# peach-xiao/EMRT

Hardware: AMD Instinct MI355X
Metric: training tiles/sec at 256x256 (higher is better)
Workload: dtype bf16; 1 GPU; EMRT ResNet50, Potsdam 256x256, 6 classes, batch 8 per GPU, fwd+bwd+SGD step (BASELINE configs[1]), bf16; global_batch=8, parallelism=dp1, hipgraph=True

## Files before the change

### emrt_amd/csrc/norm.hip

```cpp
#include "common.hpp"
#include "bn_operand.hpp"
#include <stdlib.h>

using namespace emrt;

template <class T, int MODE>
__global__ __launch_bounds__(256) void col_reduce_kernel(const T* __restrict__ x, int ldx, const T* __restrict__ dy, int lddy,
                                                         const T* __restrict__ y, int ldy, const float* __restrict__ mean,
                                                         const float* __restrict__ invstd, long long M, int C, int tx_n,
                                                         float* __restrict__ partial, long long rpb, long long bs,
                                                         double* __restrict__ dsums, float* __restrict__ facc,
                                                         const float* __restrict__ mgamma = nullptr, const float* __restrict__ mbeta = nullptr) {
  __shared__ float red[256 * 8];
  const int ty_n = 256 / tx_n;
  const int tx = threadIdx.x % tx_n, ty = threadIdx.x / tx_n;
  const int c = (blockIdx.y * tx_n + tx) * 4;
  float s0[4] = {0, 0, 0, 0}, s1[4] = {0, 0, 0, 0};
  if (c < C) {
    float mu[4] = {0, 0, 0, 0}, is[4] = {1, 1, 1, 1};
    float msc[MODE == 3 ? 4 : 1], msh[MODE == 3 ? 4 : 1];
    if (MODE == 1 || MODE == 3) {
#pragma unroll
      for (int e = 0; e < 4; ++e) { mu[e] = mean[c + e]; is[e] = invstd[c + e]; }
      if constexpr (MODE == 3) {
#pragma unroll
        for (int e = 0; e < 4; ++e) bn_scale_shift(mu[e], is[e], mgamma[c + e], mbeta[c + e], msc[e], msh[e]);
      }
    }
    for (long long r = (long long)blockIdx.x * ty_n + ty; r < M; r += (long long)gridDim.x * ty_n) {
      float v[4];
      if (MODE == 0) {
        Vec4<T>::load(x + r * ldx + c, v);
#pragma unroll
        for (int e = 0; e < 4; ++e) { s0[e] += v[e]; s1[e] = fmaf(v[e], v[e], s1[e]); }
      } else if (MODE == 1 || MODE == 3) {
        const long long rs = (long long)gridDim.x * ty_n;
        float vv[4][4], gg[4][4], oo[4][4];
#pragma unroll
        for (int u = 0; u < 4; ++u) {
          const long long ru = r + u * rs < M ? r + u * rs : r;
          Vec4<T>::load(x + ru * ldx + c, vv[u]);
          Vec4<T>::load(dy + ru * lddy + c, gg[u]);
          if (y) Vec4<T>::load(y + ru * ldy + c, oo[u]);
        }
#pragma unroll
        for (int u = 0; u < 4; ++u) {
          const bool ok = r + u * rs < M;
#pragma unroll
          for (int e = 0; e < 4; ++e) {
            float g = ok ? gg[u][e] : 0.f;
            if (y) g = oo[u][e] > 0.f ? g : 0.f;
            if constexpr (MODE == 3) g = fmaf(vv[u][e], msc[e], msh[e]) > 0.f ? g : 0.f;
            s0[e] += g;
            s1[e] = fmaf(g, (vv[u][e] - mu[e]) * is[e], s1[e]);
          }
        }
        r += 3 * rs;
      } else {
        const long long bb = (M | rpb) <= 0xffffffffll ? (long long)((unsigned)r / (unsigned)rpb) : r / rpb;
        Vec4<T>::load(x + bb * bs + (r - bb * rpb) * ldx + c, v);
#pragma unroll
        for (int e = 0; e < 4; ++e) s0[e] += v[e];
      }
    }
  }
#pragma unroll
  for (int e = 0; e < 4; ++e) { red[threadIdx.x * 8 + e] = s0[e]; red[threadIdx.x * 8 + 4 + e] = s1[e]; }
  __syncthreads();
  if (ty == 0 && c < C) {
    for (int t = 1; t < ty_n; ++t) {
#pragma unroll
      for (int e = 0; e < 4; ++e) { s0[e] += red[(t * tx_n + tx) * 8 + e]; s1[e] += red[(t * tx_n + tx) * 8 + 4 + e]; }
    }
    if (dsums) {
      double* rep = dsums + (long long)(blockIdx.x & 7) * 2 * C;
#pragma unroll
      for (int e = 0; e < 4; ++e) { atomicAdd(rep + c + e, (double)s0[e]); atomicAdd(rep + C + c + e, (double)s1[e]); }
    } else if (facc) {
#pragma unroll
      for (int e = 0; e < 4; ++e)
        if (c + e < C) atomicAdd(facc + c + e, s0[e]);
    } else {
      float* pp = partial + (long long)blockIdx.x * 2 * C;
#pragma unroll
      for (int e = 0; e < 4; ++e) { pp[c + e] = s0[e]; pp[C + c + e] = s1[e]; }
    }
  }
}

static inline void col_reduce_geometry(long long M, int C, int& tx_n, int& gx, int& gy) {
  int quads = (C + 3) / 4;
  tx_n = 64;
  while (tx_n > 1 && tx_n / 2 >= quads) tx_n /= 2;
  gy = (quads + tx_n - 1) / tx_n;
  int ty_n = 256 / tx_n;
  long long want = (M + (long long)ty_n * 8 - 1) / ((long long)ty_n * 8);
  long long cap = 512 / gy;
  if (cap < 1) cap = 1;
  gx = (int)(want < 1 ? 1 : (want > cap ? cap : want));
}

__global__ __launch_bounds__(256) void bn_sum_partials_kernel(const float* __restrict__ partial, int nblk, int C, float* __restrict__ sums ) {
  __shared__ double red[8][33];
  const int cx = threadIdx.x & 31, py = threadIdx.x >> 5;
  const int c = blockIdx.x * 32 + cx;
  double s = 0.0;
  if (c < 2 * C)
    for (int b = py; b < nblk; b += 8) s += (double)partial[(long long)b * 2 * C + c];
  red[py][cx] = s;
  __syncthreads();
  if (py == 0 && c < 2 * C) {
    double t = 0.0;
#pragma unroll
    for (int k = 0; k < 8; ++k) t += red[k][cx];
    sums[c] = (float)t;
  }
}

__global__ __launch_bounds__(256) void partials_acc_kernel(const float* __restrict__ partial, int nblk, int C, float* __restrict__ dgamma,
                                                          float* __restrict__ dbeta) {
  __shared__ double red[8][33];
  const int cx = threadIdx.x & 31, py = threadIdx.x >> 5;
  const int c = blockIdx.x * 32 + cx;
  double s = 0.0;
  if (c < 2 * C)
    for (int b = py; b < nblk; b += 8) s += (double)partial[(long long)b * 2 * C + c];
  red[py][cx] = s;
  __syncthreads();
  if (py == 0 && c < 2 * C) {
    double t = 0.0;
#pragma unroll
    for (int k = 0; k < 8; ++k) t += red[k][cx];
    if (c < C) { if (dbeta) dbeta[c] += (float)t; }
    else if (dgamma) dgamma[c - C] += (float)t;
  }
}

__global__ void bn_bwd_finalize_kernel(const float* __restrict__ sums, int C, float* __restrict__ dgamma, float* __restrict__ dbeta) {
  const int c = blockIdx.x * blockDim.x + threadIdx.x;
  if (c >= C) return;
  if (dbeta) dbeta[c] += sums[c];
  if (dgamma) dgamma[c] += sums[C + c];
}

template <class T, bool JOIN = false>
__global__ __launch_bounds__(512) void bn_apply_kernel(const T* __restrict__ x, int ldx, const T* __restrict__ res, int ldres,
                                                       T* __restrict__ y, int ldy, const double* __restrict__ sums, double inv_count,
                                                       float eps, float momentum, float* __restrict__ mean_out,
                                                       float* __restrict__ invstd_out, float* __restrict__ run_mean,
                                                       float* __restrict__ run_var, const float* __restrict__ gamma,
                                                       const float* __restrict__ beta, long long M, int C, int relu, int rows_per_pass,
                                                       BnOperand rbn) {
  const int quads = C / 4;
  const int c = (threadIdx.x % quads) * 4;
  const int lane_row = threadIdx.x / quads;
  const long long rstep = (long long)gridDim.x * rows_per_pass;
  long long r = (long long)blockIdx.x * rows_per_pass + lane_row;
  float v[4], w[4];
  if (r < M) {
    Vec4<T>::load(x + r * ldx + c, v);
    if (res) Vec4<T>::load(res + r * ldres + c, w);
  }
  extern __shared__ float bn_lds[];
  if constexpr (JOIN) bn_operand_preamble(rbn, C, bn_lds + 2 * C, blockIdx.x == 0);
  for (int ch = threadIdx.x; ch < C; ch += blockDim.x) {
    const BnChan k = bn_chan(sums, run_mean, run_var, C, ch, inv_count, eps);
    float scale, shift;
    bn_scale_shift(k.mean, k.invstd, gamma[ch], beta[ch], scale, shift);
    bn_lds[ch] = scale;
    bn_lds[C + ch] = shift;
    if (sums && blockIdx.x == 0) {
      mean_out[ch] = k.mean;
      invstd_out[ch] = k.invstd;
      if (run_mean) {
        const double mu = rep_sum(sums, C, ch) * inv_count;
        double var = rep_sum(sums, C, C + ch) * inv_count - mu * mu;
        if (var < 0.0) var = 0.0;
        run_mean[ch] = momentum * run_mean[ch] + (1.f - momentum) * (float)mu;
        run_var[ch] = momentum * run_var[ch] + (1.f - momentum) * (float)var;
      }
// ... 589 lines not shown
__global__ __launch_bounds__(256) void gn_rows_stats_kernel(const T* __restrict__ x, int ldx, long long x_bs, GnRows gr, double* __restrict__ ws,
                                                            int N, int G) {
  __shared__ float red[256][2];
  int n, l, r0, r1, HW, row0;
  gn_rows_locate(gr, n, l, r0, r1, HW, row0);
  const int g = threadIdx.x % G, rl = threadIdx.x / G, nrl = 256 / G;
  const T* xp = x + (long long)n * x_bs + (long long)row0 * ldx + g * 8;
  float s0 = 0.f, s1 = 0.f;
  for (int p = r0 + rl; p < r1; p += nrl) {
    float v[8];
    Vec8<T>::load(xp + (long long)p * ldx, v);
#pragma unroll
    for (int e = 0; e < 8; ++e) { s0 += v[e]; s1 = fmaf(v[e], v[e], s1); }
  }
  red[threadIdx.x][0] = s0; red[threadIdx.x][1] = s1;
  __syncthreads();
  if ((int)threadIdx.x < 2 * G) {
    const int gg = threadIdx.x >> 1, w = threadIdx.x & 1;
    double a = 0.0;
    for (int t = 0; t < nrl; ++t) a += (double)red[t * G + gg][w];
    atomicAdd(&ws[(((long long)l * N + n) * G + gg) * 2 + w], a);
  }
}

template <class T>
__global__ __launch_bounds__(256) void gn_rows_apply_kernel(const T* __restrict__ x, int ldx, long long x_bs, const T* __restrict__ res, int ldres,
                                                            long long res_bs, T* __restrict__ out, int ldout, long long out_bs, GnRows gr,
                                                            const double* __restrict__ ws, float* __restrict__ mean_out,
                                                            float* __restrict__ rstd_out, int N, int G, float eps, int gelu) {
  int n, l, r0, r1, HW, row0;
  gn_rows_locate(gr, n, l, r0, r1, HW, row0);
  const int g = threadIdx.x % G, rl = threadIdx.x / G, nrl = 256 / G;
  const long long sidx = ((long long)l * N + n) * G + g;
  const double cnt = (double)HW * 8.0;
  const double mu_d = ws[sidx * 2] / cnt;
  double var = ws[sidx * 2 + 1] / cnt - mu_d * mu_d;
  if (var < 0.0) var = 0.0;
  const float mu = (float)mu_d, rs = (float)(1.0 / sqrt(var + (double)eps));
  if (mean_out && r0 == 0 && rl == 0) { mean_out[sidx] = mu; rstd_out[sidx] = rs; }
  const float* gam = gn_pick<0>(gr.lv.gamma, l) + g * 8;
  const float* bet = gn_pick<0>(gr.lv.beta, l) + g * 8;
  float sc[8], sh[8];
#pragma unroll
  for (int e = 0; e < 8; ++e) { sc[e] = rs * gam[e]; sh[e] = bet[e] - mu * sc[e]; }
  const T* xp = x + (long long)n * x_bs + (long long)row0 * ldx + g * 8;
  for (int p = r0 + rl; p < r1; p += nrl) {
    float v[8], o[8];
    Vec8<T>::load(xp + (long long)p * ldx, v);
#pragma unroll
    for (int e = 0; e < 8; ++e) {
      const float u = fmaf(v[e], sc[e], sh[e]);
      o[e] = gelu ? gelu_f(u) : u;
    }
    if (res) {
      float w[8];
      Vec8<T>::load(res + (long long)n * res_bs + (long long)(row0 + p) * ldres + g * 8, w);
#pragma unroll
      for (int e = 0; e < 8; ++e) o[e] += w[e];
    }
    Vec8<T>::store(out + (long long)n * out_bs + (long long)(row0 + p) * ldout + g * 8, o);
  }
}

template <class T>
__global__ __launch_bounds__(256) void gn_rows_bwd_stats_kernel(const T* __restrict__ x, int ldx, long long x_bs, const T* __restrict__ dy, int lddy,
                                                                long long dy_bs, GnRows gr, const float* __restrict__ mean,
                                                                const float* __restrict__ rstd, double* __restrict__ ws, int N, int G, int gelu) {
  __shared__ float chs[256][17];
  int n, l, r0, r1, HW, row0;
  gn_rows_locate(gr, n, l, r0, r1, HW, row0);
  const int g = threadIdx.x % G, rl = threadIdx.x / G, nrl = 256 / G;
  const long long sidx = ((long long)l * N + n) * G + g;
  const float mu = mean[sidx], rs = rstd[sidx];
  const float* gam = gn_pick<0>(gr.lv.gamma, l);
  const float* bet = gn_pick<0>(gr.lv.beta, l);
  float ga[8], be[8];
#pragma unroll
  for (int e = 0; e < 8; ++e) { ga[e] = gam[g * 8 + e]; be[e] = bet[g * 8 + e]; }
  const T* xp = x + (long long)n * x_bs + (long long)row0 * ldx + g * 8;
  const T* gp = dy + (long long)n * dy_bs + (long long)row0 * lddy + g * 8;
  float s0[8], s1[8];
#pragma unroll
  for (int e = 0; e < 8; ++e) { s0[e] = 0.f; s1[e] = 0.f; }
  for (int p = r0 + rl; p < r1; p += nrl) {
    float v[8], d[8];
    Vec8<T>::load(xp + (long long)p * ldx, v);
    Vec8<T>::load(gp + (long long)p * lddy, d);
#pragma unroll
    for (int e = 0; e < 8; ++e) {
      const float xh = (v[e] - mu) * rs;
      const float dd = gelu ? d[e] * gelu_grad_f(xh * ga[e] + be[e]) : d[e];
      s0[e] += dd;
      s1[e] = fmaf(dd, xh, s1[e]);
    }
  }
#pragma unroll
  for (int e = 0; e < 8; ++e) { chs[threadIdx.x][e] = s0[e]; chs[threadIdx.x][8 + e] = s1[e]; }
  __syncthreads();
  const int C = G * 8;
  if ((int)threadIdx.x < C) {
    const int c = threadIdx.x, gg = c >> 3, e = c & 7;
    float a = 0.f, b = 0.f;
    for (int t = 0; t < nrl; ++t) { a += chs[t * G + gg][e]; b += chs[t * G + gg][8 + e]; }
    float* dgam = nullptr; float* dbet = nullptr;
#pragma unroll
    for (int k = 0; k < GN_MAX_LEVELS; ++k)
      if (l == k) { dgam = gr.lv.dgamma[k]; dbet = gr.lv.dbeta[k]; }
    if (dbet) atomicAdd(dbet + c, a);
    if (dgam) atomicAdd(dgam + c, b);
    float wa = gam[c] * a, wb = gam[c] * b;
#pragma unroll
    for (int o = 1; o < 8; o <<= 1) { wa += __shfl_xor(wa, o, 64); wb += __shfl_xor(wb, o, 64); }
    if (e == 0) {
      const long long si = ((long long)l * N + n) * G + gg;
      atomicAdd(&ws[si * 2], (double)wa);
      atomicAdd(&ws[si * 2 + 1], (double)wb);
    }
  }
}

template <class T>
__global__ __launch_bounds__(256) void gn_rows_bwd_dx_kernel(const T* __restrict__ x, int ldx, long long x_bs, const T* __restrict__ dy, int lddy,
                                                             long long dy_bs, T* __restrict__ dx, int lddx, long long dx_bs, GnRows gr,
                                                             const float* __restrict__ mean, const float* __restrict__ rstd,
                                                             const double* __restrict__ ws, int N, int G, int gelu) {
  int n, l, r0, r1, HW, row0;
  gn_rows_locate(gr, n, l, r0, r1, HW, row0);
  const int g = threadIdx.x % G, rl = threadIdx.x / G, nrl = 256 / G;
  const long long sidx = ((long long)l * N + n) * G + g;
  const float mu = mean[sidx], rs = rstd[sidx];
  const double inv = 1.0 / ((double)HW * 8.0);
  const float A = (float)(ws[sidx * 2] * inv), Bq = (float)(ws[sidx * 2 + 1] * inv);
  const float* gam = gn_pick<0>(gr.lv.gamma, l) + g * 8;
  const float* bet = gn_pick<0>(gr.lv.beta, l) + g * 8;
  float ga[8], be[8];
#pragma unroll
  for (int e = 0; e < 8; ++e) { ga[e] = gam[e]; be[e] = bet[e]; }
  const T* xp = x + (long long)n * x_bs + (long long)row0 * ldx + g * 8;
  const T* gp = dy + (long long)n * dy_bs + (long long)row0 * lddy + g * 8;
  for (int p = r0 + rl; p < r1; p += nrl) {
    float v[8], d[8], o[8];
    Vec8<T>::load(xp + (long long)p * ldx, v);
    Vec8<T>::load(gp + (long long)p * lddy, d);
#pragma unroll
    for (int e = 0; e < 8; ++e) {
      const float xh = (v[e] - mu) * rs;
      const float dd = gelu ? d[e] * gelu_grad_f(xh * ga[e] + be[e]) : d[e];
      o[e] = rs * (ga[e] * dd - A - xh * Bq);
    }
    Vec8<T>::store(dx + (long long)n * dx_bs + (long long)(row0 + p) * lddx + g * 8, o);
  }
}

template <class T>
__global__ __launch_bounds__(256) void ln_fwd_kernel(const T* __restrict__ a, const T* __restrict__ b, const T* __restrict__ post,
                                                     T* __restrict__ z, T* __restrict__ out, const float* __restrict__ gamma,
                                                     const float* __restrict__ beta, float* __restrict__ mean_out,
                                                     float* __restrict__ rstd_out, long long rows, int C, float eps, float pdrop,
                                                     const unsigned long long* __restrict__ seed, unsigned salt,
                                                     const T* __restrict__ qpos, int qpos_rows, T* __restrict__ q_out) {
  const int lane = threadIdx.x & 63;
  const long long row = (long long)blockIdx.x * 4 + (threadIdx.x >> 6);
  if (row >= rows) return;
  const unsigned long long sd = pdrop > 0.f ? seed[0] : 0ull;
  const float ks = pdrop > 0.f ? 1.f / (1.f - pdrop) : 1.f;
  const int nq = C / 256 + ((C % 256) ? 1 : 0);
  float v[4][4];
  float s = 0.f;
  for (int j = 0; j < nq; ++j) {
    const int c = j * 256 + lane * 4;
    if (c < C) {
      Vec4<T>::load(a + row * C + c, v[j]);
      if (b) {
        float w[4];
        Vec4<T>::load(b + row * C + c, w);
        if (pdrop > 0.f) {
          uint32_t hq[2];
          drop_quad(sd, salt, (unsigned long long)(row * C + c) >> 2, hq);
          const uint32_t thr = drop_thr16(pdrop);
#pragma unroll
          for (int e = 0; e < 4; ++e) {
            const float d = drop_quad_keep(hq, e, thr) ? w[e] * ks : 0.f;
            w[e] = to_f32(from_f32<T>(d));
          }
        }
#pragma unroll
        for (int e = 0; e < 4; ++e) v[j][e] += w[e];
      }
      if (z) {
        Vec4<T>::store(z + row * C + c, v[j]);
        if (sizeof(T) == 2) {
#pragma unroll
          for (int e = 0; e < 4; ++e) v[j][e] = to_f32(from_f32<T>(v[j][e]));
        }
      }
#pragma unroll
      for (int e = 0; e < 4; ++e) s += v[j][e];
    }
  }
  const float mu = wave_sum(s) / (float)C;
// ... 113 lines not shown
#pragma unroll
        for (int k = 0; k < R; ++k) {
          if (!ok[k]) continue;
          float o[4];
#pragma unroll
          for (int e = 0; e < 4; ++e) o[e] = rs[k] * (gd[k][j][e] - s0[k] - xh[k][j][e] * s1[k]);
          if (addend) {
            float ad[4], oa[4];
            Vec4<T>::load(addend + row[k] * C + c, ad);
#pragma unroll
            for (int e = 0; e < 4; ++e) oa[e] = o[e] + ad[e];
            Vec4<T>::store(dz + row[k] * C + c, oa);
          } else {
            Vec4<T>::store(dz + row[k] * C + c, o);
          }
          if (dzb) {
            if (pdrop > 0.f) {
              uint32_t hq[2];
              drop_quad(sd, salt, (unsigned long long)(row[k] * C + c) >> 2, hq);
              const uint32_t thr = drop_thr16(pdrop);
#pragma unroll
              for (int e = 0; e < 4; ++e)
                o[e] = drop_quad_keep(hq, e, thr) ? to_f32(from_f32<T>(o[e])) * ks : 0.f;
            }
            Vec4<T>::store(dzb + row[k] * C + c, o);
          }
        }
      }
    }
  }
#pragma unroll
  for (int j = 0; j < NQ; ++j) {
    const int c = j * 256 + lane * 4;
    if (j < nq && c < C) {
#pragma unroll
      for (int e = 0; e < 4; ++e) { sm[(wv * 2 + 0) * C + c + e] = db[j][e]; sm[(wv * 2 + 1) * C + c + e] = dg[j][e]; }
    }
  }
  __syncthreads();
  for (int c = threadIdx.x; c < C; c += TPB) {
    float b0 = 0.f, g0 = 0.f;
    for (int w = 0; w < NWV; ++w) { b0 += sm[(w * 2 + 0) * C + c]; g0 += sm[(w * 2 + 1) * C + c]; }
    if (dgamma_direct || dbeta_direct) {
      if (dbeta_direct) atomicAdd(dbeta_direct + c, b0);
      if (dgamma_direct) atomicAdd(dgamma_direct + c, g0);
    } else {
      partial[(long long)blockIdx.x * 2 * C + c] = b0;
      partial[(long long)blockIdx.x * 2 * C + C + c] = g0;
    }
  }
}

extern "C" size_t emrt_colreduce_workspace_bytes(long long M, int C) {
  int tx, gx, gy;
  col_reduce_geometry(M, C, tx, gx, gy);
  return ((size_t)gx * 2 * C + 2 * (size_t)C) * sizeof(float);
}

static inline bool bn_rowgeom(long long M, int C, int& threads, int& rows_per_pass, int& grid) {
  const int quads = C / 4;
  if (quads <= 256) { if (256 % quads) return false; threads = 256; rows_per_pass = 256 / quads; }
  else if (quads <= 512) { threads = quads; rows_per_pass = 1; }
  else return false;
  const long long per_block = (long long)(g_tune.bn_block_kb > 0 ? g_tune.bn_block_kb : 8) * 1024;
  long long g = (M * C * 2 + per_block - 1) / per_block;
  const long long gmax = (M + rows_per_pass - 1) / rows_per_pass;
  if (g < 64) g = 64;
  if (g > 4096) g = 4096;
  if (g > gmax) g = gmax;
  if (g < 1) g = 1;
  grid = (int)g;
  return true;
}

extern "C" int emrt_bn_stats(const void* x, int ldx, long long M, int C, double* sums, int dtype, void* stream) {
  EMRT_REQUIRE_TRAIN_DTYPE(dtype);
  EMRT_REQUIRE(x && sums, "null pointer");
  EMRT_REQUIRE(C % 4 == 0 && ldx % 4 == 0, "C and ld must be multiples of 4");
  int tx, gx, gy;
  col_reduce_geometry(M, C, tx, gx, gy);
  hipStream_t st = (hipStream_t)stream;
  return with_train_dtype("emrt_bn_stats", dtype, [&](auto t) {
    using T = decltype(t);
    hipLaunchKernelGGL((col_reduce_kernel<T, 0>), dim3(gx, gy), dim3(256), 0, st, (const T*)x, ldx, nullptr, 0, nullptr, 0, nullptr, nullptr, M, C, tx, nullptr, M, 0LL, sums, nullptr);
    return check_launch("emrt_bn_stats");
  });
}

extern "C" int emrt_bn_apply(const void* x, int ldx, const void* res, int ldres, void* y, int ldy, const double* sums, double count,
                             float eps, float momentum, float* mean, float* invstd, float* run_mean, float* run_var,
                             const float* gamma, const float* beta, long long M, int C, int relu, int dtype, void* stream) {
  EMRT_REQUIRE_FWD_DTYPE(dtype);
  EMRT_REQUIRE(x && y && gamma && beta, "null pointer");
  EMRT_REQUIRE(sums ? (mean && invstd) : (run_mean && run_var), "training needs mean/invstd outputs, eval needs running statistics");
  EMRT_REQUIRE(C % 4 == 0 && ldx % 4 == 0 && ldy % 4 == 0 && (!res || ldres % 4 == 0), "C and ld must be multiples of 4");
  int threads, rpp, grid;
  EMRT_REQUIRE(bn_rowgeom(M, C, threads, rpp, grid), "unsupported channel count (C/4 must divide 256, or C <= 2048)");
  hipStream_t st = (hipStream_t)stream;
  const double inv_count = sums ? 1.0 / count : 0.0;
  BnOperand none;
  memset(&none, 0, sizeof(none));
  return with_fwd_dtype("emrt_bn_apply", dtype, [&](auto t) {
    using T = decltype(t);
    hipLaunchKernelGGL((bn_apply_kernel<T>), dim3(grid), dim3(threads), (size_t)2 * C * sizeof(float), st, (const T*)x, ldx, (const T*)res, ldres, (T*)y, ldy, sums, inv_count, eps, momentum, mean, invstd, run_mean, run_var, gamma, beta, M, C, relu, rpp, none);
    return check_launch("emrt_bn_apply");
  });
}

extern "C" int emrt_bn_apply_join(const void* x, int ldx, const void* res_raw, int ldres, void* y, int ldy, const double* sums, double count,
                                  float eps, float momentum, float* mean, float* invstd, float* run_mean, float* run_var, const float* gamma,
                                  const float* beta, const double* r_sums, double r_count, float r_eps, float r_momentum, float* r_mean,
                                  float* r_invstd, float* r_run_mean, float* r_run_var, const float* r_gamma, const float* r_beta, long long M,
                                  int C, int relu, int dtype, void* stream) {
  EMRT_REQUIRE_TRAIN_DTYPE(dtype);
  EMRT_REQUIRE(x && res_raw && y && gamma && beta && sums && mean && invstd, "null pointer");
  EMRT_REQUIRE(r_sums && r_mean && r_invstd && r_gamma && r_beta && r_count > 0.0 && count > 0.0 && (r_run_mean != nullptr) == (r_run_var != nullptr),
               "the shortcut's BatchNorm needs sums, mean, invstd, gamma, beta and a positive count");
  EMRT_REQUIRE(C % 4 == 0 && ldx % 4 == 0 && ldy % 4 == 0 && ldres % 4 == 0, "C and ld must be multiples of 4");
  int threads, rpp, grid;
  EMRT_REQUIRE(bn_rowgeom(M, C, threads, rpp, grid), "unsupported channel count (C/4 must divide 256, or C <= 2048)");
  BnOperand r;
  r.sums = r_sums; r.inv_count = 1.0 / r_count; r.eps = r_eps; r.momentum = r_momentum; r.mean = r_mean; r.invstd = r_invstd;
  r.run_mean = r_run_mean; r.run_var = r_run_var; r.gamma = r_gamma; r.beta = r_beta; r.relu = 0;
  hipStream_t st = (hipStream_t)stream;
  const double inv_count = 1.0 / count;
  const size_t lds = (size_t)4 * C * sizeof(float);
  return with_train_dtype("emrt_bn_apply_join", dtype, [&](auto t) {
    using T = decltype(t);
    hipLaunchKernelGGL((bn_apply_kernel<T, true>), dim3(grid), dim3(threads), lds, st, (const T*)x, ldx, (const T*)res_raw, ldres, (T*)y, ldy, sums, inv_count, eps, momentum, mean, invstd, run_mean, run_var, gamma, beta, M, C, relu, rpp, r);
    return check_launch("emrt_bn_apply_join");
  });
}

__global__ __launch_bounds__(256) void bn_fold_kernel(const float* __restrict__ params, const float* __restrict__ buffers,
                                                      const long long* __restrict__ desc, float eps, float* __restrict__ out) {
  const long long* d = desc + 7 * (long long)blockIdx.x;
  const float* gamma = params + d[0];
  const float* beta = params + d[1];
  const float* mean = buffers + d[2];
  const float* var = buffers + d[3];
  const int C = (int)d[4];
  float* o = out + d[5];
  const float* cbias = d[6] >= 0 ? params + d[6] : nullptr;
  for (int c = threadIdx.x; c < C; c += blockDim.x) {
    const float sc = gamma[c] * rsqrtf(var[c] + eps);
    o[c] = sc;
    o[C + c] = beta[c] + ((cbias ? cbias[c] : 0.f) - mean[c]) * sc;
  }
}
extern "C" int emrt_bn_fold(const float* params, const float* buffers, const long long* desc, int n, float eps, float* out, void* stream) {
  EMRT_REQUIRE(params && buffers && desc && out && n > 0, "null pointer");
  hipLaunchKernelGGL(bn_fold_kernel, dim3(n), dim3(256), 0, (hipStream_t)stream, params, buffers, desc, eps, out);
  return check_launch("emrt_bn_fold");
}

extern "C" int emrt_bn_bwd_reduce(const void* x, int ldx, const void* dy, int lddy, const void* y, int ldy, const float* mean,
                                  const float* invstd, long long M, int C, double* sums, const float* mask_gamma, const float* mask_beta,
                                  int dtype, void* stream) {
  EMRT_REQUIRE_TRAIN_DTYPE(dtype);
  EMRT_REQUIRE(x && dy && mean && invstd && sums, "null pointer");
  EMRT_REQUIRE((mask_gamma != nullptr) == (mask_beta != nullptr) && !(mask_beta && y), "mask_gamma and mask_beta come together and replace y");
  EMRT_REQUIRE(C % 4 == 0 && ldx % 4 == 0 && lddy % 4 == 0 && (!y || ldy % 4 == 0), "C and ld must be multiples of 4");
  int tx, gx, gy;
  col_reduce_geometry(M, C, tx, gx, gy);
  hipStream_t st = (hipStream_t)stream;
  return with_train_dtype("emrt_bn_bwd_reduce", dtype, [&](auto t) {
    using T = decltype(t);
    if (mask_beta) {
      hipLaunchKernelGGL((col_reduce_kernel<T, 3>), dim3(gx, gy), dim3(256), 0, st, (const T*)x, ldx, (const T*)dy, lddy, (const T*)nullptr, 0, mean, invstd, M, C, tx, nullptr, M, 0LL, sums, nullptr, mask_gamma, mask_beta);
      return check_launch("emrt_bn_bwd_reduce");
    }
    hipLaunchKernelGGL((col_reduce_kernel<T, 1>), dim3(gx, gy), dim3(256), 0, st, (const T*)x, ldx, (const T*)dy, lddy, (const T*)y, ldy, mean, invstd, M, C, tx, nullptr, M, 0LL, sums, nullptr);
    return check_launch("emrt_bn_bwd_reduce");
  });
}

extern "C" int emrt_bn_bwd_dx(const void* x, int ldx, const void* dy, int lddy, const void* y, int ldy, void* dx, int lddx,
                              void* dres, int lddres, const float* mean, const float* invstd, const float* gamma,
                              const double* sums, const double* local_sums, double count, float* dgamma, float* dbeta, long long M,
                              int C, const float* beta_y_moments, int sums_vs_x, const float* mask_beta, int dtype, void* stream) {
  EMRT_REQUIRE_TRAIN_DTYPE(dtype);
  EMRT_REQUIRE(x && dy && dx && mean && invstd && gamma && sums, "null pointer");
  EMRT_REQUIRE(!(mask_beta && (y || beta_y_moments || sums_vs_x)), "mask_beta (ReLU mask re-derived from x) excludes y and the fused-sum forms");
  EMRT_REQUIRE(C % 4 == 0 && ldx % 4 == 0 && lddy % 4 == 0 && lddx % 4 == 0, "C and ld must be multiples of 4");
  int threads, rpp, grid;
  EMRT_REQUIRE(bn_rowgeom(M, C, threads, rpp, grid), "unsupported channel count (C/4 must divide 256, or C <= 2048)");
  hipStream_t st = (hipStream_t)stream;
  return with_train_dtype("emrt_bn_bwd_dx", dtype, [&](auto t) {
    using T = decltype(t);
    if (mask_beta) {
      hipLaunchKernelGGL((bn_bwd_dx_kernel<T, true>), dim3(grid), dim3(threads), (size_t)2 * C * sizeof(float), st, (const T*)x, ldx, (const T*)dy, lddy, (const T*)nullptr, 0, (T*)dx, lddx, (T*)dres, lddres, mean, invstd, gamma, sums, local_sums, 1.0 / count, dgamma, dbeta, M, C, rpp, nullptr, 0, mask_beta);
      return check_launch("emrt_bn_bwd_dx");
    }
    hipLaunchKernelGGL((bn_bwd_dx_kernel<T>), dim3(grid), dim3(threads), (size_t)2 * C * sizeof(float), st, (const T*)x, ldx, (const T*)dy, lddy, (const T*)y, ldy, (T*)dx, lddx, (T*)dres, lddres, mean, invstd, gamma, sums, local_sums, 1.0 / count, dgamma, dbeta, M, C, rpp, beta_y_moments, sums_vs_x, mask_beta);
    return check_launch("emrt_bn_bwd_dx");
  });
}

template <class T>
__global__ __launch_bounds__(256) void colsum_scalar_kernel(const T* __restrict__ x, int ldx, long long rpb, long long bs, long long M,
                                                            float* __restrict__ dbias) {
  __shared__ float red[4];
  const int c = blockIdx.x;
  float s = 0.f;
  for (long long r = threadIdx.x; r < M; r += 256) {
    const long long bb = r / rpb;
    s += to_f32(x[bb * bs + (r - bb * rpb) * ldx + c]);
  }
  s = wave_sum(s);
  if ((threadIdx.x & 63) == 0) red[threadIdx.x >> 6] = s;
  __syncthreads();
  if (threadIdx.x == 0) dbias[c] += red[0] + red[1] + red[2] + red[3];
}

extern "C" int emrt_colsum_acc(const void* x, int ldx, long long rows_per_batch, long long x_bs, long long M, int C, float* dbias,
                               void* workspace, int dtype, void* stream) {
  EMRT_REQUIRE_TRAIN_DTYPE(dtype);
  EMRT_REQUIRE(rows_per_batch > 0, "bad batch geometry");
  EMRT_REQUIRE(x && dbias && workspace, "null pointer");
  return with_train_dtype("emrt_colsum_acc", dtype, [&](auto t) {
    using T = decltype(t);
    if (C % 4 != 0 || ldx % 4 != 0 || x_bs % 4 != 0) {
      hipStream_t st0 = (hipStream_t)stream;
      hipLaunchKernelGGL((colsum_scalar_kernel<T>), dim3(C), dim3(256), 0, st0, (const T*)x, ldx, rows_per_batch, x_bs, M, dbias);
      return check_launch("emrt_colsum_acc(scalar)");
    }
    int tx, gx, gy;
    col_reduce_geometry(M, C, tx, gx, gy);
    hipStream_t st = (hipStream_t)stream;
    float* partial = (float*)workspace;
    const bool direct = g_tune.ln_atomic != 0;
    hipLaunchKernelGGL((col_reduce_kernel<T, 2>), dim3(gx, gy), dim3(256), 0, st, (const T*)x, ldx, nullptr, 0, nullptr, 0, nullptr, nullptr, M, C, tx, partial, rows_per_batch, x_bs, nullptr, direct ? dbias : nullptr);
    if (!direct) hipLaunchKernelGGL(partials_acc_kernel, dim3((C + 31) / 32), dim3(256), 0, st, partial, gx, C, (float*)nullptr, dbias);
    return check_launch("emrt_colsum_acc");
  });
}

struct ColsumLevelsArgs {
  const void* x[8];
  int T, L, B, Lv, C;
  int start[4], count[4];
  float* dst;
};
template <class T>
__global__ __launch_bounds__(256) void colsum_levels_kernel(ColsumLevelsArgs a) {
  const int quads = a.C / 4;
  const int cq = threadIdx.x % quads, lane_row = threadIdx.x / quads, lanes = 256 / quads;
  const int l = blockIdx.y;
  float acc[4] = {0.f, 0.f, 0.f, 0.f};
  const int npair = a.T * a.B;
  for (int r = blockIdx.x * lanes + lane_row; r < a.count[l]; r += gridDim.x * lanes) {
    const long long row = a.start[l] + r;
    for (int p0 = blockIdx.z; p0 < npair; p0 += 4 * gridDim.z) {
      float v[4][4];
#pragma unroll
      for (int u = 0; u < 4; ++u) {
        const int pp = p0 + u * gridDim.z;
        const int t = pp < npair ? pp / a.B : 0, b = pp < npair ? pp - t * a.B : 0;
        Vec4<T>::load((const T*)a.x[t] + ((long long)b * a.Lv + row) * a.C + cq * 4, v[u]);
        if (pp >= npair) { v[u][0] = 0.f; v[u][1] = 0.f; v[u][2] = 0.f; v[u][3] = 0.f; }
      }
#pragma unroll
      for (int u = 0; u < 4; ++u)
#pragma unroll
        for (int e = 0; e < 4; ++e) acc[e] += v[u][e];
    }
  }
  __shared__ float red[256 * 4];
#pragma unroll
  for (int e = 0; e < 4; ++e) red[(lane_row * quads + cq) * 4 + e] = acc[e];
  __syncthreads();
  for (int c = threadIdx.x; c < a.C; c += 256) {
    float s = 0.f;
    for (int q = 0; q < lanes; ++q) s += red[(q * quads + c / 4) * 4 + (c & 3)];
    atomicAdd(a.dst + (long long)l * a.C + c, s);
  }
}

extern "C" int emrt_colsum_levels_multi(const void* const* xs, int T, const int* level_start, const int* level_count, int L, int B, int Lv, int C,
                                        float* dst, int dtype, void* stream) {
  EMRT_REQUIRE_TRAIN_DTYPE(dtype);
  EMRT_REQUIRE(xs && level_start && level_count && dst, "null pointer");
  EMRT_REQUIRE(T >= 1 && T <= 8 && L >= 1 && L <= 4 && B > 0 && Lv > 0, "1..8 tensors, 1..4 levels");
  EMRT_REQUIRE(C % 4 == 0 && C / 4 <= 256 && 256 % (C / 4) == 0, "C / 4 must divide 256");
  ColsumLevelsArgs a;
  memset(&a, 0, sizeof(a));
  int most = 0;
  for (int t = 0; t < T; ++t) {
    EMRT_REQUIRE(xs[t] && ((uintptr_t)xs[t]) % 16 == 0, "null or unaligned tensor");
    a.x[t] = xs[t];
  }
  for (int l = 0; l < L; ++l) {
    EMRT_REQUIRE(level_start[l] >= 0 && level_count[l] > 0 && level_start[l] + level_count[l] <= Lv, "level outside the token axis");
    a.start[l] = level_start[l]; a.count[l] = level_count[l];
    most = level_count[l] > most ? level_count[l] : most;
  }
  a.T = T; a.L = L; a.B = B; a.Lv = Lv; a.C = C; a.dst = dst;
  const int lanes = 256 / (C / 4);
  int gx = (most + lanes - 1) / lanes;
  if (gx > 64) gx = 64;
  const int gz = T * B >= 8 ? 4 : 1;
  hipStream_t st = (hipStream_t)stream;
  return with_train_dtype("emrt_colsum_levels_multi", dtype, [&](auto t) {
    using E = decltype(t);
    hipLaunchKernelGGL((colsum_levels_kernel<E>), dim3(gx, L, gz), dim3(256), 0, st, a);
    return check_launch("emrt_colsum_levels_multi");
  });
}

#define EMRT_MAX_BNGROUP 8
struct BnGroupArgs { EmrtBnGroupDesc d[EMRT_MAX_BNGROUP]; int first[EMRT_MAX_BNGROUP + 1]; int n; };

__device__ __forceinline__ int bn_group_pick(const BnGroupArgs& g, int& local, int& nblk) {
  int i = 0;
  for (int k = 1; k < g.n; ++k) i += (int)blockIdx.x >= g.first[k] ? 1 : 0;
// ... 185 lines not shown
    return check_launch("emrt_bn_group_bwd");
  });
}

static inline bool gn_use_fused(int HW, int C, int G) {
  const int cpg = C / G;
  return HW <= 4096 && cpg % 4 == 0 && cpg / 4 <= 64 && 256 % (cpg / 4) == 0 && (cpg / 4) * 64 >= 64;
}

static inline int gn_geom(int HW, int C, int* pix_per_block) {
  const int lanes = 256 / (C / 4);
  int ppb = lanes * 8;
  int blocks = (HW + ppb - 1) / ppb;
  if (blocks > 64) { blocks = 64; ppb = (HW + 63) / 64; ppb = (ppb + lanes - 1) / lanes * lanes; blocks = (HW + ppb - 1) / ppb; }
  *pix_per_block = ppb;
  return blocks;
}

extern "C" int emrt_groupnorm_fwd(const void* x, int ldx, long long x_bs, const void* res, int ldres, long long res_bs, void* out,
                                  int ldout, long long out_bs, const float* gamma, const float* beta, float* mean, float* rstd,
                                  double* workspace, int N, int HW, int C, int G, float eps, int gelu, int dtype, void* stream) {
  EMRT_REQUIRE_FWD_DTYPE(dtype);
  EMRT_REQUIRE(x && out && gamma && beta && workspace, "null pointer");
  EMRT_REQUIRE(C % 4 == 0 && (C / 4) <= 256 && 256 % (C / 4) == 0 && G > 0 && G <= 256 && C % G == 0 && (C / G) % 4 == 0, "unsupported C/G");
  EMRT_REQUIRE(ldx % 4 == 0 && ldout % 4 == 0 && x_bs % 4 == 0 && out_bs % 4 == 0, "strides must be multiples of 4");
  hipStream_t st = (hipStream_t)stream;
  return with_fwd_dtype("emrt_groupnorm_fwd", dtype, [&](auto t) {
    using T = decltype(t);
    if (gn_use_fused(HW, C, G)) {
      hipLaunchKernelGGL((gn_fused_fwd_kernel<T>), dim3(N * G), dim3(256), 0, st, (const T*)x, ldx, x_bs, (const T*)res, ldres, res_bs, (T*)out, ldout, out_bs, gamma, beta, mean, rstd, HW, C, G, eps, gelu);
      return check_launch("emrt_groupnorm_fwd");
    }
    int ppb;
    const int blocks = gn_geom(HW, C, &ppb);
    hipLaunchKernelGGL((gn_stats_kernel<T>), dim3(blocks, N), dim3(256), 0, st, (const T*)x, ldx, x_bs, workspace, HW, C, G, ppb);
    hipLaunchKernelGGL((gn_apply_kernel<T>), dim3(blocks, N), dim3(256), 0, st, (const T*)x, ldx, x_bs, (const T*)res, ldres, res_bs, (T*)out, ldout, out_bs, gamma, beta, workspace, mean, rstd, HW, C, G, eps, gelu, ppb);
    return check_launch("emrt_groupnorm_fwd");
  });
}

extern "C" int emrt_groupnorm_bwd(const void* x, int ldx, long long x_bs, const void* dy, int lddy, long long dy_bs, void* dx,
                                  int lddx, long long dx_bs, const float* gamma, const float* beta, const float* mean,
                                  const float* rstd, float* dgamma, float* dbeta, double* workspace, int N, int HW, int C, int G,
                                  int gelu, int dtype, void* stream) {
  EMRT_REQUIRE_TRAIN_DTYPE(dtype);
  EMRT_REQUIRE(x && dy && dx && gamma && beta && mean && rstd && workspace, "null pointer");
  EMRT_REQUIRE(C % 4 == 0 && (C / 4) <= 256 && 256 % (C / 4) == 0 && G > 0 && G <= 256 && C % G == 0 && (C / G) % 4 == 0, "unsupported C/G");
  hipStream_t st = (hipStream_t)stream;
  return with_train_dtype("emrt_groupnorm_bwd", dtype, [&](auto t) {
    using T = decltype(t);
    if (gn_use_fused(HW, C, G)) {
      hipLaunchKernelGGL((gn_fused_bwd_kernel<T>), dim3(N * G), dim3(256), 0, st, (const T*)x, ldx, x_bs, (const T*)dy, lddy, dy_bs, (T*)dx, lddx, dx_bs, gamma, beta, mean, rstd, dgamma, dbeta, HW, C, G, gelu);
      return check_launch("emrt_groupnorm_bwd");
    }
    int ppb;
    const int blocks = gn_geom(HW, C, &ppb);
    hipLaunchKernelGGL((gn_bwd_reduce_kernel<T>), dim3(blocks, N), dim3(256), 0, st, (const T*)x, ldx, x_bs, (const T*)dy, lddy, dy_bs, gamma, beta, mean, rstd, workspace, HW, C, G, gelu, ppb);
    const size_t lds = (size_t)2 * G * sizeof(float);
    hipLaunchKernelGGL((gn_bwd_dx_kernel<T>), dim3(blocks, N), dim3(256), lds, st, (const T*)x, ldx, x_bs, (const T*)dy, lddy, dy_bs, (T*)dx, lddx, dx_bs, gamma, beta, mean, rstd, workspace, dgamma, dbeta, HW, C, G, gelu, ppb);
    return check_launch("emrt_groupnorm_bwd");
  });
}

extern "C" int emrt_layernorm_fwd(const void* a, const void* b, const void* post, void* z, void* out, const float* gamma,
                                  const float* beta, float* mean, float* rstd, long long rows, int C, float eps, float pdrop,
                                  const unsigned long long* seed, unsigned salt, const void* qpos, int qpos_rows, void* q_out, int dtype, void* stream) {
  EMRT_REQUIRE_FWD_DTYPE(dtype);
  EMRT_REQUIRE(a && out && gamma && beta, "null pointer");
  EMRT_REQUIRE((q_out == nullptr) == (qpos == nullptr) && (!q_out || (qpos_rows > 0 && q_out != out)), "q_out needs qpos [qpos_rows][C] and a buffer of its own");
  EMRT_REQUIRE(pdrop >= 0.f && pdrop < 1.f && (pdrop == 0.f || (seed && b)), "dropout needs 0 <= p < 1, a device seed and a branch input b");
  EMRT_REQUIRE(C % 4 == 0 && C <= 1024, "C must be a multiple of 4 and <= 1024");
  hipStream_t st = (hipStream_t)stream;
  const int grid = (int)((rows + 3) / 4);
  return with_fwd_dtype("emrt_layernorm_fwd", dtype, [&](auto t) {
    using T = decltype(t);
    hipLaunchKernelGGL((ln_fwd_kernel<T>), dim3(grid), dim3(256), 0, st, (const T*)a, (const T*)b, (const T*)post, (T*)z, (T*)out, gamma, beta, mean, rstd, rows, C, eps, pdrop, seed, salt, (const T*)qpos, qpos_rows, (T*)q_out);
    return check_launch("emrt_layernorm_fwd");
  });
}

static inline bool ln_bwd_wide(int C) { return C <= 256 && g_tune.ln_bwd_threads >= 512; }
static inline long long ln_bwd_blocks(long long rows, int C) {
  const bool wide = ln_bwd_wide(C);
  const int per = g_tune.ln_bwd_rows > 0 ? g_tune.ln_bwd_rows : (wide ? 64 : 32);
  const int cap = g_tune.ln_bwd_max_blocks > 0 ? g_tune.ln_bwd_max_blocks : (wide ? 256 : 512);
  long long blocks = (rows + per - 1) / per;
  if (blocks > cap) blocks = cap;
  if (blocks < 1) blocks = 1;
  return blocks;
}

extern "C" size_t emrt_layernorm_bwd_workspace_bytes(long long rows, int C) {
  return ((size_t)(ln_bwd_blocks(rows, C) + 1) * 2 * C + 2 * (size_t)C) * sizeof(float);
}

extern "C" int emrt_layernorm_bwd(const void* z, const void* dy, void* dz, const float* gamma, const float* mean, const float* rstd,
                                  float* dgamma, float* dbeta, long long rows, int C, void* workspace, void* dz_branch, float pdrop,
                                  const unsigned long long* seed, unsigned salt, const void* dz_addend, const void* dy2, void* dysum, int dtype, void* stream) {
  EMRT_REQUIRE_TRAIN_DTYPE(dtype);
  EMRT_REQUIRE(z && dy && dz && gamma && mean && rstd && workspace, "null pointer");
  EMRT_REQUIRE(!dysum || (dy2 && dysum != dz && dysum != dy && dysum != dy2), "dysum (= dy + dy2) needs dy2 and a buffer of its own");
  EMRT_REQUIRE(pdrop >= 0.f && pdrop < 1.f && (pdrop == 0.f || (seed && dz_branch)), "dropout needs 0 <= p < 1, a device seed and dz_branch");
  EMRT_REQUIRE(!dz_addend || dz_addend != dz, "dz_addend must not alias dz");
  EMRT_REQUIRE(C % 4 == 0 && C <= 1024, "C must be a multiple of 4 and <= 1024");
  long long blocks = ln_bwd_blocks(rows, C);
  int rpb = (int)((rows + blocks - 1) / blocks);
  const bool small = C <= 256;
  const bool wide = ln_bwd_wide(C);
  const int step = wide ? 32 : small ? 16 : 8;
  rpb = (rpb + step - 1) / step * step;
  blocks = (rows + rpb - 1) / rpb;
  float* partial = (float*)workspace;
  const bool direct = (dgamma || dbeta) && g_tune.ln_atomic != 0;
  const size_t lds = (size_t)(wide ? 16 : 8) * C * sizeof(float);
  hipStream_t st = (hipStream_t)stream;
  return with_train_dtype("emrt_layernorm_bwd", dtype, [&](auto t) {
    using T = decltype(t);
    auto launch = [&](auto* kernel, int threads) {
      hipLaunchKernelGGL(kernel, dim3((unsigned)blocks), dim3(threads), lds, st, (const T*)z, (const T*)dy, (T*)dz, gamma, mean, rstd, partial, rows, C, rpb, (T*)dz_branch, pdrop, seed, salt, direct ? dgamma : nullptr, direct ? dbeta : nullptr, (const T*)dz_addend, (const T*)dy2, (T*)dysum);
    };
    if (wide) launch(dy2 ? ln_bwd_kernel<T, 4, 1, 512, true> : ln_bwd_kernel<T, 4, 1, 512, false>, 512);
    else if (small) launch(dy2 ? ln_bwd_kernel<T, 4, 1, 256, true> : ln_bwd_kernel<T, 4, 1, 256, false>, 256);
    else launch(dy2 ? ln_bwd_kernel<T, 2, 4, 256, true> : ln_bwd_kernel<T, 2, 4, 256, false>, 256);
    if (!direct) hipLaunchKernelGGL(partials_acc_kernel, dim3((2 * C + 31) / 32), dim3(256), 0, st, partial, (int)blocks, C, dgamma, dbeta);
    return check_launch("emrt_layernorm_bwd");
  });
}

static int gn_fill_levels(GnLevels& lv, const int* level_start, const int* level_hw, int L, const float* const* gamma, const float* const* beta,
                          float* const* dgamma, float* const* dbeta) {
  if (L < 1 || L > GN_MAX_LEVELS) return -1;
  lv.L = L;
  for (int l = 0; l < GN_MAX_LEVELS; ++l) {
    const int s = l < L ? l : 0;
    lv.start[l] = level_start[s]; lv.hw[l] = level_hw[s];
    lv.gamma[l] = gamma[s]; lv.beta[l] = beta[s];
    lv.dgamma[l] = dgamma ? dgamma[s] : nullptr; lv.dbeta[l] = dbeta ? dbeta[s] : nullptr;
    if (!lv.gamma[l] || !lv.beta[l] || lv.hw[l] < 1 || lv.hw[l] > 4096 || lv.start[l] < 0) return -1;
  }
  return 0;
}

static int gn_rows_plan(GnRows& gr, int rows_per_block) {
  gr.rows_per_block = rows_per_block;
  gr.per_image = 0;
  for (int l = 0; l < GN_MAX_LEVELS; ++l) {
    gr.nblk[l] = l < gr.lv.L ? (gr.lv.hw[l] + rows_per_block - 1) / rows_per_block : 0;
    gr.per_image += gr.nblk[l];
  }
  return gr.per_image;
}
static inline bool gn_rows_ok(int C, int G, int ld0, int ld1, int ld2, long long bs0, long long bs1, long long bs2) {
  return C == 8 * G && 256 % G == 0 && C <= 256 && ld0 % 8 == 0 && ld1 % 8 == 0 && ld2 % 8 == 0 && bs0 % 8 == 0 && bs1 % 8 == 0 && bs2 % 8 == 0;
}

extern "C" int emrt_groupnorm_levels_fwd(const void* x, int ldx, long long x_bs, const void* res, int ldres, long long res_bs, void* out,
                                         int ldout, long long out_bs, const float* const* gamma, const float* const* beta, float* mean,
                                         float* rstd, const int* level_start, const int* level_hw, int L, int N, int C, int G, float eps,
                                         int gelu, double* stat_ws, int dtype, void* stream) {
  EMRT_REQUIRE_FWD_DTYPE(dtype);
  EMRT_REQUIRE(x && out && gamma && beta && level_start && level_hw, "null pointer");
  EMRT_REQUIRE(G > 0 && C % G == 0 && gn_use_fused(1, C, G), "unsupported C / G for the one-block-per-group kernel");
  EMRT_REQUIRE(ldx % 4 == 0 && ldout % 4 == 0 && x_bs % 4 == 0 && out_bs % 4 == 0 && (!res || (ldres % 4 == 0 && res_bs % 4 == 0)), "strides must be multiples of 4");
  GnLevels lv;
  EMRT_REQUIRE(gn_fill_levels(lv, level_start, level_hw, L, gamma, beta, nullptr, nullptr) == 0, "1..4 levels of at most 4096 rows");
  hipStream_t st = (hipStream_t)stream;
  return with_fwd_dtype("emrt_groupnorm_levels_fwd", dtype, [&](auto t) {
    using T = decltype(t);
// ... 39 lines not shown
```

Baseline: 998.9 tiles/s.

## Split BN backward reduce into dedicated kernel with prefetch and 8-wide loads

Moves the batch-norm backward column reduction out of the generic col_reduce kernel into its own kernel. The new kernel uses 8-element vector loads for aligned bf16 data, software-prefetches the next row group while the current one is computed, reduces across lanes with shuffles before the shared-memory step, and gets its own grid geometry with a higher block cap. The goal is to hide memory latency and raise bandwidth on this bandwidth-bound pass. The GroupNorm row backward gets the same one-row prefetch, and the LayerNorm backward rows-per-block choice changes for small row counts. These add register pressure and more double atomics per launch.

```diff
diff --git a/emrt_amd/csrc/norm.hip b/emrt_amd/csrc/norm.hip
--- a/emrt_amd/csrc/norm.hip
+++ b/emrt_amd/csrc/norm.hip
@@ -1,61 +1,26 @@
 #include "common.hpp"
 #include "bn_operand.hpp"
 #include <stdlib.h>
+#include <type_traits>
 
 using namespace emrt;
 
 template <class T, int MODE>
-__global__ __launch_bounds__(256) void col_reduce_kernel(const T* __restrict__ x, int ldx, const T* __restrict__ dy, int lddy,
-                                                         const T* __restrict__ y, int ldy, const float* __restrict__ mean,
-                                                         const float* __restrict__ invstd, long long M, int C, int tx_n,
+__global__ __launch_bounds__(256) void col_reduce_kernel(const T* __restrict__ x, int ldx, long long M, int C, int tx_n,
                                                          float* __restrict__ partial, long long rpb, long long bs,
-                                                         double* __restrict__ dsums, float* __restrict__ facc,
-                                                         const float* __restrict__ mgamma = nullptr, const float* __restrict__ mbeta = nullptr) {
+                                                         double* __restrict__ dsums, float* __restrict__ facc) {
   __shared__ float red[256 * 8];
   const int ty_n = 256 / tx_n;
   const int tx = threadIdx.x % tx_n, ty = threadIdx.x / tx_n;
   const int c = (blockIdx.y * tx_n + tx) * 4;
   float s0[4] = {0, 0, 0, 0}, s1[4] = {0, 0, 0, 0};
   if (c < C) {
-    float mu[4] = {0, 0, 0, 0}, is[4] = {1, 1, 1, 1};
-    float msc[MODE == 3 ? 4 : 1], msh[MODE == 3 ? 4 : 1];
-    if (MODE == 1 || MODE == 3) {
-#pragma unroll
-      for (int e = 0; e < 4; ++e) { mu[e] = mean[c + e]; is[e] = invstd[c + e]; }
-      if constexpr (MODE == 3) {
-#pragma unroll
-        for (int e = 0; e < 4; ++e) bn_scale_shift(mu[e], is[e], mgamma[c + e], mbeta[c + e], msc[e], msh[e]);
-      }
-    }
     for (long long r = (long long)blockIdx.x * ty_n + ty; r < M; r += (long long)gridDim.x * ty_n) {
       float v[4];
       if (MODE == 0) {
         Vec4<T>::load(x + r * ldx + c, v);
 #pragma unroll
         for (int e = 0; e < 4; ++e) { s0[e] += v[e]; s1[e] = fmaf(v[e], v[e], s1[e]); }
-      } else if (MODE == 1 || MODE == 3) {
-        const long long rs = (long long)gridDim.x * ty_n;
-        float vv[4][4], gg[4][4], oo[4][4];
-#pragma unroll
-        for (int u = 0; u < 4; ++u) {
-          const long long ru = r + u * rs < M ? r + u * rs : r;
-          Vec4<T>::load(x + ru * ldx + c, vv[u]);
-          Vec4<T>::load(dy + ru * lddy + c, gg[u]);
-          if (y) Vec4<T>::load(y + ru * ldy + c, oo[u]);
-        }
-#pragma unroll
-        for (int u = 0; u < 4; ++u) {
-          const bool ok = r + u * rs < M;
-#pragma unroll
-          for (int e = 0; e < 4; ++e) {
-            float g = ok ? gg[u][e] : 0.f;
-            if (y) g = oo[u][e] > 0.f ? g : 0.f;
-            if constexpr (MODE == 3) g = fmaf(vv[u][e], msc[e], msh[e]) > 0.f ? g : 0.f;
-            s0[e] += g;
-            s1[e] = fmaf(g, (vv[u][e] - mu[e]) * is[e], s1[e]);
-          }
-        }
-        r += 3 * rs;
       } else {
         const long long bb = (M | rpb) <= 0xffffffffll ? (long long)((unsigned)r / (unsigned)rpb) : r / rpb;
         Vec4<T>::load(x + bb * bs + (r - bb * rpb) * ldx + c, v);
@@ -96,6 +61,134 @@
   int ty_n = 256 / tx_n;
   long long want = (M + (long long)ty_n * 8 - 1) / ((long long)ty_n * 8);
   long long cap = 512 / gy;
+  if (cap < 1) cap = 1;
+  gx = (int)(want < 1 ? 1 : (want > cap ? cap : want));
+}
+
+constexpr int BNR_U = 2;
+template <class T, int V>
+struct RowRaw;
+template <>
+struct RowRaw<float, 4> {
+  float4 v;
+  __device__ __forceinline__ void load(const float* p) { v = *reinterpret_cast<const float4*>(p); }
+  __device__ __forceinline__ void get(float (&o)[4]) const { o[0] = v.x; o[1] = v.y; o[2] = v.z; o[3] = v.w; }
+};
+template <>
+struct RowRaw<float, 8> {
+  float4 a, b;
+  __device__ __forceinline__ void load(const float* p) { a = *reinterpret_cast<const float4*>(p); b = *reinterpret_cast<const float4*>(p + 4); }
+  __device__ __forceinline__ void get(float (&o)[8]) const { o[0] = a.x; o[1] = a.y; o[2] = a.z; o[3] = a.w; o[4] = b.x; o[5] = b.y; o[6] = b.z; o[7] = b.w; }
+};
+template <class T>
+struct RowRaw<T, 4> {
+  uint2 v;
+  __device__ __forceinline__ void load(const T* p) { v = *reinterpret_cast<const uint2*>(p); }
+  __device__ __forceinline__ void get(float (&o)[4]) const {
+    T t;
+    t.v = (unsigned short)(v.x & 0xffffu); o[0] = to_f32(t); t.v = (unsigned short)(v.x >> 16); o[1] = to_f32(t);
+    t.v = (unsigned short)(v.y & 0xffffu); o[2] = to_f32(t); t.v = (unsigned short)(v.y >> 16); o[3] = to_f32(t);
+  }
+};
+template <class T>
+struct RowRaw<T, 8> {
+  uint4 v;
+  __device__ __forceinline__ void load(const T* p) { v = *reinterpret_cast<const uint4*>(p); }
+  __device__ __forceinline__ void get(float (&o)[8]) const { Vec8<T>::unpack(v, o); }
+};
+
+template <class T, int MASK, int V>
+__global__ __launch_bounds__(256) void bn_bwd_reduce_kernel(const T* __restrict__ x, int ldx, const T* __restrict__ dy, int lddy,
+                                                            const T* __restrict__ y, int ldy, const float* __restrict__ mean,
+                                                            const float* __restrict__ invstd, long long M, int C, int tx_n,
+                                                            double* __restrict__ dsums, const float* __restrict__ mgamma,
+                                                            const float* __restrict__ mbeta) {
+  constexpr int U = BNR_U;
+  __shared__ float red[4 * 64 * 2 * V];
+  const int ty_n = 256 / tx_n;
+  const int tx = threadIdx.x % tx_n, ty = threadIdx.x / tx_n;
+  const int c = (blockIdx.y * tx_n + tx) * V;
+  float s0[V], s1[V];
+#pragma unroll
+  for (int e = 0; e < V; ++e) { s0[e] = 0.f; s1[e] = 0.f; }
+  if (c < C) {
+    float mu[V], is[V];
+    float msc[MASK == 2 ? V : 1], msh[MASK == 2 ? V : 1];
+#pragma unroll
+    for (int e = 0; e < V; ++e) {
+      mu[e] = mean[c + e]; is[e] = invstd[c + e];
+      if constexpr (MASK == 2) bn_scale_shift(mu[e], is[e], mgamma[c + e], mbeta[c + e], msc[e], msh[e]);
+    }
+    const long long rs = (long long)gridDim.x * ty_n;
+    RowRaw<T, V> xa[U], ga[U], ya[MASK == 1 ? U : 1];
+#define BNR_LOAD(r_)                                                            \
+  _Pragma("unroll") for (int u = 0; u < U; ++u) {                               \
+    const long long ru = (r_) + u * rs < M ? (r_) + u * rs : M - 1;             \
+    xa[u].load(x + ru * ldx + c);                                               \
+    ga[u].load(dy + ru * lddy + c);                                             \
+    if constexpr (MASK == 1) ya[u].load(y + ru * ldy + c);                      \
+  }
+    long long r = (long long)blockIdx.x * ty_n + ty;
+    BNR_LOAD(r)
+    while (r < M) {
+      float vv[U][V], gg[U][V], oo[MASK == 1 ? U : 1][V];
+#pragma unroll
+      for (int u = 0; u < U; ++u) {
+        xa[u].get(vv[u]); ga[u].get(gg[u]);
+        if constexpr (MASK == 1) ya[u].get(oo[u]);
+      }
+      const long long rn = r + U * rs;
+      BNR_LOAD(rn)
+#pragma unroll
+      for (int u = 0; u < U; ++u) {
+        const bool ok = r + u * rs < M;
+#pragma unroll
+        for (int e = 0; e < V; ++e) {
+          float g = ok ? gg[u][e] : 0.f;
+          if constexpr (MASK == 1) g = oo[u][e] > 0.f ? g : 0.f;
+          if constexpr (MASK == 2) g = fmaf(vv[u][e], msc[e], msh[e]) > 0.f ? g : 0.f;
+          s0[e] += g;
+          s1[e] = fmaf(g, (vv[u][e] - mu[e]) * is[e], s1[e]);
+        }
+      }
+      r = rn;
+    }
+#undef BNR_LOAD
+  }
+  for (int o = tx_n; o < 64; o <<= 1) {
+#pragma unroll
+    for (int e = 0; e < V; ++e) { s0[e] += __shfl_xor(s0[e], o, 64); s1[e] += __shfl_xor(s1[e], o, 64); }
+  }
+  const int lane = threadIdx.x & 63, wv = threadIdx.x >> 6;
+  if (lane < tx_n) {
+#pragma unroll
+    for (int e = 0; e < V; ++e) { red[(wv * 64 + lane) * 2 * V + e] = s0[e]; red[(wv * 64 + lane) * 2 * V + V + e] = s1[e]; }
+  }
+  __syncthreads();
+  double* rep = dsums + (long long)(blockIdx.x & 7) * 2 * C;
+  const int ncol = tx_n * V;
+  for (int i = threadIdx.x; i < 2 * ncol; i += 256) {
+    const int which = i >= ncol, j = i - which * ncol;
+    const int t = j / V, e = j % V;
+    const int cc = blockIdx.y * ncol + j;
+    if (cc < C) {
+      float a = 0.f;
+#pragma unroll
+      for (int w = 0; w < 4; ++w) a += red[(w * 64 + t) * 2 * V + which * V + e];
+      atomicAdd(rep + which * C + cc, (double)a);
+    }
+  }
+}
+
+constexpr int BNR_TRIPS = 4;
+static inline void bn_reduce_geometry(long long M, int C, int V, int& tx_n, int& gx, int& gy) {
+  const int vecs = C / V;
+  tx_n = 64;
+  while (tx_n > 1 && tx_n / 2 >= vecs) tx_n /= 2;
+  gy = (vecs + tx_n - 1) / tx_n;
+  const long long per = (long long)(256 / tx_n) * BNR_U * BNR_TRIPS;
+  const long long want = (M + per - 1) / per;
+  long long cap = 2048 / gy;
   if (cap < 1) cap = 1;
   gx = (int)(want < 1 ? 1 : (want > cap ? cap : want));
 }
@@ -851,10 +944,17 @@
   float s0[8], s1[8];
 #pragma unroll
   for (int e = 0; e < 8; ++e) { s0[e] = 0.f; s1[e] = 0.f; }
-  for (int p = r0 + rl; p < r1; p += nrl) {
+  int p = r0 + rl;
+  RowRaw<T, 8> xa, da;
+  {
+    const int pc = p < r1 ? p : r0;
+    xa.load(xp + (long long)pc * ldx); da.load(gp + (long long)pc * lddy);
+  }
+  for (; p < r1; p += nrl) {
     float v[8], d[8];
-    Vec8<T>::load(xp + (long long)p * ldx, v);
-    Vec8<T>::load(gp + (long long)p * lddy, d);
+    xa.get(v); da.get(d);
+    const int pn = p + nrl < r1 ? p + nrl : p;
+    xa.load(xp + (long long)pn * ldx); da.load(gp + (long long)pn * lddy);
 #pragma unroll
     for (int e = 0; e < 8; ++e) {
       const float xh = (v[e] - mu) * rs;
@@ -880,11 +980,7 @@
     float wa = gam[c] * a, wb = gam[c] * b;
 #pragma unroll
     for (int o = 1; o < 8; o <<= 1) { wa += __shfl_xor(wa, o, 64); wb += __shfl_xor(wb, o, 64); }
-    if (e == 0) {
-      const long long si = ((long long)l * N + n) * G + gg;
-      atomicAdd(&ws[si * 2], (double)wa);
-      atomicAdd(&ws[si * 2 + 1], (double)wb);
-    }
+    if (e < 2) atomicAdd(&ws[(((long long)l * N + n) * G + gg) * 2 + e], (double)(e ? wb : wa));
   }
 }
 
@@ -1164,7 +1260,7 @@
   hipStream_t st = (hipStream_t)stream;
   return with_train_dtype("emrt_bn_stats", dtype, [&](auto t) {
     using T = decltype(t);
-    hipLaunchKernelGGL((col_reduce_kernel<T, 0>), dim3(gx, gy), dim3(256), 0, st, (const T*)x, ldx, nullptr, 0, nullptr, 0, nullptr, nullptr, M, C, tx, nullptr, M, 0LL, sums, nullptr);
+    hipLaunchKernelGGL((col_reduce_kernel<T, 0>), dim3(gx, gy), dim3(256), 0, st, (const T*)x, ldx, M, C, tx, nullptr, M, 0LL, sums, nullptr);
     return check_launch("emrt_bn_stats");
   });
 }
@@ -1243,17 +1339,29 @@
   EMRT_REQUIRE(x && dy && mean && invstd && sums, "null pointer");
   EMRT_REQUIRE((mask_gamma != nullptr) == (mask_beta != nullptr) && !(mask_beta && y), "mask_gamma and mask_beta come together and replace y");
   EMRT_REQUIRE(C % 4 == 0 && ldx % 4 == 0 && lddy % 4 == 0 && (!y || ldy % 4 == 0), "C and ld must be multiples of 4");
-  int tx, gx, gy;
-  col_reduce_geometry(M, C, tx, gx, gy);
+  if (M < 1) return 0;
   hipStream_t st = (hipStream_t)stream;
   return with_train_dtype("emrt_bn_bwd_reduce", dtype, [&](auto t) {
     using T = decltype(t);
-    if (mask_beta) {
-      hipLaunchKernelGGL((col_reduce_kernel<T, 3>), dim3(gx, gy), dim3(256), 0, st, (const T*)x, ldx, (const T*)dy, lddy, (const T*)nullptr, 0, mean, invstd, M, C, tx, nullptr, M, 0LL, sums, nullptr, mask_gamma, mask_beta);
+    auto launch = [&](auto vtag) {
+      constexpr int V = decltype(vtag)::value;
+      int tx, gx, gy;
+      bn_reduce_geometry(M, C, V, tx, gx, gy);
+      const dim3 grid(gx, gy);
+      if (mask_beta)
+        hipLaunchKernelGGL((bn_bwd_reduce_kernel<T, 2, V>), grid, dim3(256), 0, st, (const T*)x, ldx, (const T*)dy, lddy, (const T*)nullptr, 0, mean, invstd, M, C, tx, sums, mask_gamma, mask_beta);
+      else if (y)
+        hipLaunchKernelGGL((bn_bwd_reduce_kernel<T, 1, V>), grid, dim3(256), 0, st, (const T*)x, ldx, (const T*)dy, lddy, (const T*)y, ldy, mean, invstd, M, C, tx, sums, (const float*)nullptr, (const float*)nullptr);
+      else
+        hipLaunchKernelGGL((bn_bwd_reduce_kernel<T, 0, V>), grid, dim3(256), 0, st, (const T*)x, ldx, (const T*)dy, lddy, (const T*)nullptr, 0, mean, invstd, M, C, tx, sums, (const float*)nullptr, (const float*)nullptr);
       return check_launch("emrt_bn_bwd_reduce");
-    }
-    hipLaunchKernelGGL((col_reduce_kernel<T, 1>), dim3(gx, gy), dim3(256), 0, st, (const T*)x, ldx, (const T*)dy, lddy, (const T*)y, ldy, mean, invstd, M, C, tx, nullptr, M, 0LL, sums, nullptr);
-    return check_launch("emrt_bn_bwd_reduce");
+    };
+    if constexpr (sizeof(T) == 2) {
+      const bool v8 = C % 8 == 0 && ldx % 8 == 0 && lddy % 8 == 0 && (!y || ldy % 8 == 0) &&
+                      (((uintptr_t)x | (uintptr_t)dy | (uintptr_t)y) & 15) == 0;
+      if (v8) return launch(std::integral_constant<int, 8>{});
+    }
+    return launch(std::integral_constant<int, 4>{});
   });
 }
 
@@ -1312,7 +1420,7 @@
     hipStream_t st = (hipStream_t)stream;
     float* partial = (float*)workspace;
     const bool direct = g_tune.ln_atomic != 0;
-    hipLaunchKernelGGL((col_reduce_kernel<T, 2>), dim3(gx, gy), dim3(256), 0, st, (const T*)x, ldx, nullptr, 0, nullptr, 0, nullptr, nullptr, M, C, tx, partial, rows_per_batch, x_bs, nullptr, direct ? dbias : nullptr);
+    hipLaunchKernelGGL((col_reduce_kernel<T, 2>), dim3(gx, gy), dim3(256), 0, st, (const T*)x, ldx, M, C, tx, partial, rows_per_batch, x_bs, nullptr, direct ? dbias : nullptr);
     if (!direct) hipLaunchKernelGGL(partials_acc_kernel, dim3((C + 31) / 32), dim3(256), 0, st, partial, gx, C, (float*)nullptr, dbias);
     return check_launch("emrt_colsum_acc");
   });
@@ -1664,8 +1772,8 @@
 static inline bool ln_bwd_wide(int C) { return C <= 256 && g_tune.ln_bwd_threads >= 512; }
 static inline long long ln_bwd_blocks(long long rows, int C) {
   const bool wide = ln_bwd_wide(C);
-  const int per = g_tune.ln_bwd_rows > 0 ? g_tune.ln_bwd_rows : (wide ? 64 : 32);
   const int cap = g_tune.ln_bwd_max_blocks > 0 ? g_tune.ln_bwd_max_blocks : (wide ? 256 : 512);
+  const int per = g_tune.ln_bwd_rows > 0 ? g_tune.ln_bwd_rows : (wide && rows > 32ll * cap ? 64 : 32);
   long long blocks = (rows + per - 1) / per;
   if (blocks > cap) blocks = cap;
   if (blocks < 1) blocks = 1;
```

Result: no change. 1006 tiles/s (median of 6 runs) (+0.7%).
